# kyprifog/ballista

Hardware: AMD Instinct MI355X
Metric: tpch_q1_sf100_rows_per_sec (higher is better)
Workload: dtype f64

## Files before the change

ballista_amd/csrc/host/capi.cpp:

```cpp
#include <cstdio>
#include <cstring>

#include "../util_kernels.h"
#include "plan.hpp"

using namespace bhip;

#define BHIP_API_BEGIN try {
#define BHIP_API_END                                              \
    return BHIP_OK;                                               \
    }                                                             \
    catch (const bhip::Error& e) {                                \
        bhip::set_last_error(e.what());                           \
        return e.code;                                            \
    }                                                             \
    catch (const std::bad_alloc&) {                               \
        bhip::set_last_error("host allocation failed");           \
        return BHIP_EOOM;                                         \
    }                                                             \
    catch (const std::exception& e) {                             \
        bhip::set_last_error(std::string("internal error: ") + e.what()); \
        return BHIP_EINVAL;                                       \
    }                                                             \
    catch (...) {                                                 \
// ... 510 lines not shown
    h->ex = Exec{ctx, ctx->acquire_stream()};
    h->s = p->p->execute(partition, h->ex);
    *out = h.release();
    trace_point("plan_execute: leave");
    BHIP_API_END
}

bhip_status bhip_plan_collect(bhip_plan* p, int32_t cap, bhip_batch** out, int32_t* n_out) {
    BHIP_API_BEGIN
    need(p, "plan"); need(out, "out"); need(n_out, "n_out");
    ContextPtr ctx = p->p->context();
    if (!ctx) fail(BHIP_EEXEC, "Ballista Error: this plan has unresolved leaves and no device context; it can be inspected, not executed");
    ctx->set_device();
    trace_point("plan_collect: enter");
    std::vector<BatchPtr> got;
    {
        const Exec ex{ctx, ctx->acquire_stream()};
        struct Release { const Exec& ex; ~Release() { ex.ctx->release_stream(ex.stream); } } release{ex};
        const int n_parts = p->p->output_partitioning().count;
        for (int part = 0; part < n_parts; ++part) {
            StreamPtr s = p->p->execute(part, ex);
            while (BatchPtr b = s->next()) got.push_back(b);
        }
        ctx->wait_stream(ex.stream);
    }
    if ((int64_t)got.size() > cap) fail(BHIP_EINVAL, "bhip_plan_collect: the plan yields " + std::to_string(got.size()) + " batches, the caller has room for " + std::to_string(cap));
    for (size_t i = 0; i < got.size(); ++i) out[i] = wrap_batch(got[i]);
    *n_out = (int32_t)got.size();
    trace_point("plan_collect: leave");
    BHIP_API_END
}

bhip_status bhip_stream_next(bhip_stream* s, bhip_batch** out) {
    BHIP_API_BEGIN
    need(s, "stream"); need(out, "out");
    s->ex.ctx->set_device();
    trace_point("stream_next: enter");
    BatchPtr b = s->s->next();
    trace_point("stream_next: operators returned");
    if (b) s->ex.ctx->wait_stream(s->ex.stream);
    *out = b ? wrap_batch(b) : nullptr;
    trace_point("stream_next: leave");
    BHIP_API_END
}

bhip_status bhip_stream_schema(const bhip_stream* s, int32_t cap, const char** names, int32_t* dtypes, int32_t* nullable, int32_t* n_cols) {
    BHIP_API_BEGIN
    need(s, "stream");
    fill_schema(*s->s->schema(), nullptr, cap, names, dtypes, nullable, n_cols);
    BHIP_API_END
}

void bhip_stream_release(bhip_stream* s) { delete s; }

bhip_status bhip_stream_drain(bhip_stream* s, bhip_batch_sink sink, void* user, uint64_t* num_rows, uint64_t* num_batches, uint64_t* num_bytes) {
    BHIP_API_BEGIN
    need(s, "stream");
    s->ex.ctx->set_device();
    uint64_t rows = 0, batches = 0, bytes = 0;
    while (BatchPtr b = s->s->next()) {
        s->ex.ctx->wait_stream(s->ex.stream);
        rows += (uint64_t)b->n_rows;
        batches += 1;
// ... 202 lines not shown
```

ballista_amd/csrc/host/core.hpp:

```cpp
#pragma once
#include <hip/hip_runtime.h>
#include <atomic>
#include <cstdint>
#include <cstring>
#include <map>
#include <memory>
#include <mutex>
#include <stdexcept>
#include <string>
#include <vector>

#include "../../../include/ballista_hip.h"
#include "../kernels.h"

namespace bhip {

struct Error : std::runtime_error {
    bhip_status code;
    Error(bhip_status c, const std::string& m) : std::runtime_error(m), code(c) {}
};
[[noreturn]] inline void fail(bhip_status c, const std::string& m) { throw Error(c, m); }
inline void hip_check(hipError_t e, const char* what) {
    if (e != hipSuccess) {
        if (e == hipErrorOutOfMemory) fail(BHIP_EOOM, std::string(what) + ": " + hipGetErrorString(e));
// ... 60 lines not shown
    int device_;
    int cus_ = 256;
    int timing_ = 0;
    std::mutex mu_;
    std::multimap<size_t, Block> free_blocks_;
    std::map<void*, Block> live_;
    uint64_t in_use_ = 0, peak_ = 0, cached_ = 0;
    std::vector<hipStream_t> stream_pool_;
    static constexpr size_t N_SLOTS = 1024;
    struct HostSlot { volatile uint64_t w[8]; };
    HostSlot* slots_ = nullptr;
    std::atomic<uint64_t> slot_seq_{0};
    bool spin_wait_ = true;
    double k_ms_ = 0;
    uint64_t k_launches_ = 0;
    std::string k_name_, k_variant_, k_key_form_, k_sort_limit_form_, k_join_key_form_, k_nested_loop_form_, k_join_probe_form_;
    struct PendingTimed { hipEvent_t a, b; const char* name; uint64_t bytes; };
    std::vector<PendingTimed> pending_timed_;
    std::vector<hipEvent_t> event_pool_;
    std::map<std::string, KernelStat> k_stats_;
};
using ContextPtr = std::shared_ptr<Context>;

struct Exec {
    ContextPtr ctx;
    hipStream_t stream;
    LaunchCfg cfg() const { return LaunchCfg{ctx->cus(), stream}; }
};

struct KernelTimer {
    const Exec& ex;
    const char* name;
    hipEvent_t a = nullptr, b = nullptr;
    uint64_t bytes = 0;
    KernelTimer(const Exec& e, const char* n, int64_t rows = -1, uint64_t algorithmic_bytes = 0) : ex(e), name(n), bytes(algorithmic_bytes) {
        const int level = ex.ctx->timing_level();
        if (level <= 0 || (level == 1 && rows < (1 << 18))) return;
        a = ex.ctx->timing_event();
        b = ex.ctx->timing_event();
        hipEventRecord(a, ex.stream);
    }
    void stop() {
        if (!a) return;
        hipEventRecord(b, ex.stream);
        ex.ctx->push_timed(a, b, name, bytes);
        a = b = nullptr;
    }
    ~KernelTimer() { stop(); }
};
// ... 94 lines not shown
struct Field {
    std::string name;
    int dtype;
    bool nullable;
    bool large = false;
    bool binary = false;
};

struct Schema {
    std::vector<Field> fields;
    int index_of(const std::string& name) const {
        for (size_t i = 0; i < fields.size(); ++i)
            if (fields[i].name == name) return (int)i;
        return -1;
    }
};
using SchemaPtr = std::shared_ptr<const Schema>;

struct Batch {
    SchemaPtr schema;
    std::vector<Column> cols;
    int64_t n_rows = 0;
    ContextPtr ctx;
    int64_t memory_size() const;
};
using BatchPtr = std::shared_ptr<const Batch>;

BatchPtr batch_from_host(const ContextPtr& ctx, int n_cols, const bhip_column_desc* cols, int64_t n_rows, bool device_ptrs);
void column_to_host(const Batch& b, int i, void* data, int32_t* offsets, uint8_t* validity);
BatchPtr batch_from_text(const ContextPtr& ctx, int format, const void* text_host, int64_t n_bytes, int n_fields,
                         const bhip_column_desc* fields, int n_proj, const int32_t* projection, const bhip_csv_opts& csv_opts);

void* pinned_host_alloc(size_t bytes);
void pinned_host_free(void* p, size_t bytes);

BatchPtr take_batch(const Exec& ex, const Batch& in, const uint32_t* indices, int64_t n_out, SchemaPtr schema = nullptr,
                    bool permutation = false);
Column take_column(const Exec& ex, const Column& c, const uint32_t* indices, int64_t n_out, int64_t known_bytes = -1);
BatchPtr concat_batches(const Exec& ex, const SchemaPtr& schema, const std::vector<BatchPtr>& parts);
BatchPtr slice_head(const Exec& ex, const Batch& in, int64_t n);

void trace_point(const char* what);

template <class T>
T read_device(const Exec& ex, const T* dev) {
    T host;
// ... 15 lines not shown
```

ballista_amd/csrc/host/ops_agg.cpp:

```cpp
#include "../sort_kernels.h"
#include "../util_kernels.h"
#include "hash_kernels.h"
#include "plan.hpp"
#include "sop.hpp"

namespace bhip {

static int sum_type(int t) {
    if (dt_is_float(t)) return t;
    if (dt_is_unsigned(t)) return DT_UINT64;
    return DT_INT64;
}

static int minmax_kind(int t, bool is_min) {
    if (dt_is_float(t)) return is_min ? ACC_MIN_F64 : ACC_MAX_F64;
    if (dt_is_unsigned(t)) return is_min ? ACC_MIN_U64 : ACC_MAX_U64;
    return is_min ? ACC_MIN_I64 : ACC_MAX_I64;
}

static const char* lowcard_launch_name(int gmax, bool batches) {
    if (batches) return gmax == 1 ? "scan_agg_lowcard_g1_batches" : gmax == 4 ? "scan_agg_lowcard_g4_batches" : "scan_agg_lowcard_g8_batches";
    return gmax == 1 ? "scan_agg_lowcard_g1" : gmax == 4 ? "scan_agg_lowcard_g4" : "scan_agg_lowcard_g8";
}

// ... 376 lines not shown
            if (g->kind != BHIP_EXPR_COLUMN) continue;
            const int ci = src_schema.index_of(g->name);
            if (ci < 0 || b0.cols[ci].dtype != DT_UTF8 || b0.cols[ci].data_bytes <= 2 * b0.n_rows) continue;
            Temp t2(ex);
            uint32_t* dev = t2.get<uint32_t>(1);
            TIMED_LAUNCH(ex, "utf8_max_len", launch_utf8_max_len(ex.cfg(), b0.cols[ci].offsets->as<int32_t>(), std::min<int64_t>(b0.n_rows, 65536), dev));
            longest = std::max(longest, read_device(ex, dev));
        }
        if (longest > 3) use_lean = false;
        if (longest > 7) use_sop = false;
    }
    const KeyLayout* key_layout = &pb.key_info();

    Temp tmp(ex);
    const LaunchCfg cfg = ex.cfg();
    TailInfo* info = tmp.get<TailInfo>(1);
    ScanStatus* status = &info->st;
    uint64_t* totals = group_.size() <= (size_t)TAIL_TOTALS ? info->totals : tmp.get<uint64_t>(group_.size() + 1);
    GroupRec* table = nullptr;
    int64_t n_groups = 0;
    TimedLaunches timer(ex);

    auto alloc_columns = [&](const KeyLayout& kinfo, int64_t n) { return alloc_emit_columns(ex, out_schema, kinfo, group_.size(), emits, nullable, n); };
    auto emit_table = [&](const GroupRec* tab, int64_t n_alloc, const ScanStatus* dev_n, const KeyLayout& kinfo) {
        EmitColumns E = alloc_columns(kinfo, n_alloc);
        if (dev_n && n_alloc <= EMIT_ALL_MAX_GROUPS && group_.size() <= (size_t)EMIT_ALL_MAX_KEYS && emits.size() <= (size_t)EMIT_ALL_MAX_VALUES) {
            EmitAllArgs A = emit_all_args(E, totals);
            A.table = tab;
            A.status = dev_n;
            TIMED_LAUNCH(ex, "emit_all", launch_emit_all(cfg, A));
            return E;
        }
        for (size_t gi = 0; gi < group_.size(); ++gi) {
            const Column& c = E.out->cols[gi];
            const EmitKeySpec& ks = E.key[gi];
            uint64_t* vptr = validity_of(c);
            if (c.dtype != DT_UTF8) {
                if (n_alloc) TIMED_LAUNCH(ex, "emit_group_key", launch_emit_group_key(cfg, tab, n_alloc, ks, c.data->ptr(), vptr, nullptr, dev_n));
            } else if (n_alloc > 0 && n_alloc <= EMIT_UTF8_SMALL_MAX) {
                TIMED_LAUNCH(ex, "emit_group_utf8_small", launch_emit_group_utf8_small(cfg, tab, n_alloc, ks, vptr, c.offsets->as<int32_t>(),
                                                       c.data->as<uint8_t>(), totals + gi, dev_n));
            } else {
                uint32_t* lengths = tmp.get<uint32_t>((size_t)n_alloc + 1);
                void* scan_tmp = tmp.get<uint8_t>(exclusive_scan_temp_bytes(n_alloc));
                if (n_alloc) TIMED_LAUNCH(ex, "emit_group_key", launch_emit_group_key(cfg, tab, n_alloc, ks, nullptr, vptr, lengths));
                HIP_CHECK(exclusive_scan_u32_i32(ex.stream, lengths, n_alloc, c.offsets->as<int32_t>(), true, totals + gi, scan_tmp));
                if (n_alloc) TIMED_LAUNCH(ex, "emit_group_utf8", launch_emit_group_utf8(cfg, tab, n_alloc, ks, c.offsets->as<int32_t>(), c.data->as<uint8_t>()));
            }
        }
        EmitValueBatch vb;
        vb.n = 0;
        for (size_t k = 0; k < emits.size(); ++k) {
// ... 158 lines not shown
        early = EmitColumns();
        GroupRec id;
        memset(&id, 0, sizeof(id));
        for (int i = 0; i < n_acc; ++i) {
            switch (P0.acc[i].kind) {
                case ACC_MIN_F64:
                case ACC_MAX_F64: { double v = __builtin_nan(""); memcpy(&id.acc[i], &v, 8); } break;
                case ACC_MIN_I64: id.acc[i] = (uint64_t)INT64_MAX; break;
                case ACC_MAX_I64: id.acc[i] = (uint64_t)INT64_MIN; break;
                case ACC_MIN_U64: id.acc[i] = UINT64_MAX; break;
                case ACC_MAX_U64: id.acc[i] = 0; break;
                default: break;
            }
        }
        table = tmp.get<GroupRec>(1);
        HIP_CHECK(hipMemcpyAsync(table, &id, sizeof(id), hipMemcpyHostToDevice, ex.stream));
        stream_wait(ex);
        n_groups = 1;
    }

    trace_point("aggregate: done");
    if (early.out) {
        finish_table(early, n_groups, tail.totals);
        return {early.out};
    }
    const EmitColumns out = slots.valid ? emit_slots(slots, n_groups) : emit_table(table, n_groups, nullptr, *key_layout);
    if (!out.utf8_cols.empty()) {
        std::vector<uint64_t> host(group_.size() + 1);
        if (group_.size() <= (size_t)TAIL_TOTALS) {
            const TailInfo ti = read_device(ex, info);
            for (size_t i = 0; i < group_.size(); ++i) host[i] = ti.totals[i];
        } else {
            HIP_CHECK(hipMemcpyAsync(host.data(), totals, group_.size() * 8, hipMemcpyDeviceToHost, ex.stream));
            stream_wait(ex);
        }
        finish_table(out, n_groups, host.data());
    }
    return {out.out};
}

}
```

ballista_amd/csrc/host/ops_sort.cpp:

```cpp
#include "../sort_kernels.h"
#include "../topk_kernels.h"
#include "../util_kernels.h"
#include "plan.hpp"

namespace bhip {

void radix_sort_pairs(const Exec& ex, BufferPtr& keys, BufferPtr& perm, int64_t n) {
    if (n <= 1) return;
    const LaunchCfg cfg = ex.cfg();
    if (n <= small_sort_max()) {
        HIP_CHECK(small_sort_pairs(cfg, keys->as<uint64_t>(), perm->as<uint32_t>(), n));
        return;
    }
    Temp tmp(ex);
    uint64_t* diff_dev = tmp.get<uint64_t>(1);
    HIP_CHECK(radix_key_diff(cfg, keys->as<uint64_t>(), n, diff_dev));
    const uint64_t diff = read_device(ex, diff_dev);
    if (diff == 0) return;
    BufferPtr keys2 = make_buffer(ex, (size_t)n * 8 + 8), perm2 = make_buffer(ex, (size_t)n * 4 + 8);
    void* pass_tmp = tmp.get<uint8_t>(radix_sort_temp_bytes(n));
    for (int byte = 0; byte < 8; ++byte) {
        if (((diff >> (8 * byte)) & 0xFF) == 0) continue;
        HIP_CHECK(radix_pass(cfg, keys->as<uint64_t>(), perm->as<uint32_t>(), n, byte, keys2->as<uint64_t>(),
                             perm2->as<uint32_t>(), pass_tmp));
// ... 4 lines not shown

SortExec::SortExec(std::vector<SortDesc> exprs, PlanPtr input) : exprs_(std::move(exprs)) {
    input_ = std::move(input);
    ctx_ = input_->context();
    Utf8Lowering low(*input_->schema());
    for (auto& s : exprs_) {
        expr_type(s.expr, *input_->schema());
        low.rewrite(s.expr, true);
    }
    low.validate();
}
PlanPtr SortExec::with_new_children(const std::vector<PlanPtr>& c) const {
    if (c.size() != 1) fail(BHIP_EINVAL, "SortExec wrong number of children");
    return std::make_shared<SortExec>(exprs_, c[0]);
}
std::string SortExec::describe() const {
    std::string s = "SortExec: [";
    for (size_t i = 0; i < exprs_.size(); ++i)
        s += (i ? ", " : "") + exprs_[i].expr->to_string() + (exprs_[i].descending ? " DESC" : " ASC") +
             (exprs_[i].nulls_first ? " NULLS FIRST" : " NULLS LAST");
    return s + "]";
}

StreamPtr SortExec::execute(int partition, const Exec& ex) const {
    if (partition != 0) fail(BHIP_EINVAL, "SortExec invalid partition " + std::to_string(partition));
    if (input_->output_partitioning().count != 1) fail(BHIP_EINVAL, "SortExec requires a single input partition");
    auto self = std::static_pointer_cast<const SortExec>(shared_from_this());
    return StreamPtr(new LazyStream(schema(), [self, ex]() -> std::vector<BatchPtr> {
        std::vector<BatchPtr> parts;
        {
            auto s = self->input_->execute(0, ex);
            while (BatchPtr b = s->next())
                if (b->n_rows > 0) parts.push_back(b);
        }
        if (parts.empty()) return {};
        trace_point("sort: input ready");
        BatchPtr in = concat_batches(ex, self->schema(), parts);
        const int64_t n = in->n_rows;
        const LaunchCfg cfg = ex.cfg();
        static const bool no_rowsort = env_flag("BHIP_NO_ROWSORT");
        if (!no_rowsort && n <= ROWSORT_MAX_ROWS && self->exprs_.size() <= (size_t)ROWSORT_MAX_KEYS && in->cols.size() <= (size_t)ROWSORT_MAX_COLS) {
            RowSortArgs A;
            memset(&A, 0, sizeof(A));
            A.n_rows = (int32_t)n;
            A.n_keys = (int32_t)self->exprs_.size();
            A.n_cols = (int32_t)in->cols.size();
            std::vector<Column> key_cols;
            for (size_t k = 0; k < self->exprs_.size(); ++k) {
                const SortDesc& sd = self->exprs_[k];
                key_cols.push_back(evaluate_column(ex, *in, sd.expr));
                A.key[k] = key_cols.back().ref();
                A.desc[k] = sd.descending ? 1 : 0;
                A.nulls_first[k] = sd.nulls_first ? 1 : 0;
            }
            auto out = std::make_shared<Batch>();
            out->schema = in->schema;
            out->ctx = in->ctx;
            out->n_rows = n;
            for (size_t ci = 0; ci < in->cols.size(); ++ci) {
// ... 320 lines not shown
```

ballista_amd/csrc/host/plan.hpp:

```cpp
#pragma once
#include <functional>
#include <mutex>

#include "../util_kernels.h"
#include "core.hpp"
#include "expr.hpp"

namespace bhip {

struct Partitioning {
    int scheme = BHIP_PART_UNKNOWN;
    int count = 1;
    std::vector<ExprPtr> exprs;
};

class RecordBatchStream {
public:
    virtual ~RecordBatchStream() = default;
    virtual SchemaPtr schema() const = 0;
    virtual BatchPtr next() = 0;
};
using StreamPtr = std::unique_ptr<RecordBatchStream>;

class ExecutionPlan;
// ... 124 lines not shown

class MergeExec : public UnaryExec {
public:
    explicit MergeExec(PlanPtr input);
    const char* name() const override { return "MergeExec"; }
    SchemaPtr schema() const override { return input_->schema(); }
    Partitioning output_partitioning() const override { return Partitioning{BHIP_PART_UNKNOWN, 1, {}}; }
    PlanPtr with_new_children(const std::vector<PlanPtr>& c) const override;
    StreamPtr execute(int partition, const Exec& ex) const override;
};

class LimitExec : public UnaryExec {
public:
    LimitExec(PlanPtr input, int64_t limit, bool global);
    const char* name() const override { return global_ ? "GlobalLimitExec" : "LocalLimitExec"; }
    SchemaPtr schema() const override { return input_->schema(); }
    Partitioning output_partitioning() const override;
    PlanPtr with_new_children(const std::vector<PlanPtr>& c) const override;
    StreamPtr execute(int partition, const Exec& ex) const override;
    std::string describe() const override { return std::string(name()) + ": limit=" + std::to_string(limit_); }
private:
    int64_t limit_;
    bool global_;
};

class HashAggregateExec : public UnaryExec {
public:
    HashAggregateExec(int mode, std::vector<std::pair<ExprPtr, std::string>> group_exprs,
                      std::vector<AggregateDesc> aggr, PlanPtr input);
    const char* name() const override { return "HashAggregateExec"; }
    SchemaPtr schema() const override { return schema_; }
    PlanPtr with_new_children(const std::vector<PlanPtr>& c) const override;
    StreamPtr execute(int partition, const Exec& ex) const override;
    std::string describe() const override;
private:
    std::vector<BatchPtr> run(int partition, const Exec& ex) const;
    std::vector<BatchPtr> run_packed(int partition, const Exec& ex, const HashAggregateExec* as_final = nullptr) const;
    std::vector<BatchPtr> run_wide(int partition, const Exec& ex) const;
    bool run_single_partial(const Exec& ex, std::vector<BatchPtr>& out) const;
    std::vector<BatchPtr> run_strings(int partition, const Exec& ex) const;
    bool strings_ = false;
    int mode_;
    std::vector<std::pair<ExprPtr, std::string>> group_;
    std::vector<AggregateDesc> aggr_;
    SchemaPtr schema_;
    mutable std::atomic<int> path_hint_{0};
// ... 182 lines not shown
```

ballista_amd/csrc/kernels_sort.hip:

```cpp
#include <hip/hip_runtime.h>
#include <stdlib.h>
#include "sort_device.h"
#include "sort_kernels.h"
#include "util_kernels.h"
#include "vm_device.h"

namespace bhip {

constexpr int SORT_BLOCK = 256;
constexpr int SORT_ITEMS = 16;
constexpr int SORT_CHUNK = SORT_BLOCK * SORT_ITEMS;

constexpr int SORT_ITEMS_SMALL = 4;
static int sort_items_for(int64_t n) {
    static const int forced = env_int("BHIP_SORT_ITEMS", 0);
    if (forced == SORT_ITEMS_SMALL || forced == SORT_ITEMS) return forced;
    return n <= (1ll << 21) ? SORT_ITEMS_SMALL : SORT_ITEMS;
}

template <int ITEMS>
__global__ void __launch_bounds__(SORT_BLOCK)
radix_hist_kernel(const uint64_t* keys, int64_t n, int shift, uint32_t* hist, int n_blocks) {
    __shared__ uint32_t s_hist[256];
    s_hist[threadIdx.x] = 0;
// ... 442 lines not shown
#define BSORT_TAIL(W_)                                                                                                                 \
    {                                                                                                                                  \
        hipLaunchKernelGGL(bsort_scatter_kernel<W_>, dim3(g), dim3(SORT_BLOCK), 0, cfg.stream, words, digits, n, first, fill, records);  \
        hipLaunchKernelGGL(bsort_rank_kernel<W_>, dim3(g), dim3(SORT_BLOCK), 0, cfg.stream, records, n, first, bins, perm, status);      \
    }
    switch (W) {
        case 1: BSORT_HEAD(1) break;
        case 2: BSORT_HEAD(2) break;
        case 3: BSORT_HEAD(3) break;
        default: BSORT_HEAD(4) break;
    }
    if ((e = exclusive_scan_u32_u32(cfg.stream, bins, (int64_t)n_bins, first, false, nullptr, scan_tmp)) != hipSuccess) return e;
    switch (W) {
        case 1: BSORT_TAIL(1) break;
        case 2: BSORT_TAIL(2) break;
        case 3: BSORT_TAIL(3) break;
        default: BSORT_TAIL(4) break;
    }
#undef BSORT_HEAD
#undef BSORT_TAIL
    return hipGetLastError();
}

__device__ inline int rowsort_cmp_key(const ColumnRef& c, uint32_t a, uint32_t b) {
    if (c.dtype == DT_UTF8) {
        const int32_t oa = c.offsets[a], ob = c.offsets[b];
        const int la = c.offsets[a + 1] - oa, lb = c.offsets[b + 1] - ob;
        const uint8_t* sa = reinterpret_cast<const uint8_t*>(c.data) + oa;
        const uint8_t* sb = reinterpret_cast<const uint8_t*>(c.data) + ob;
        const int m = la < lb ? la : lb;
        for (int p = 0; p < m; ++p)
            if (sa[p] != sb[p]) return sa[p] < sb[p] ? -1 : 1;
        for (int p = m; p < la; ++p) if (sa[p] != 0) return 1;
        for (int p = m; p < lb; ++p) if (sb[p] != 0) return -1;
        return la < lb ? -1 : la > lb ? 1 : 0;
    }
    const uint64_t ka = fixed_key_image(c, a), kb = fixed_key_image(c, b);
    return ka < kb ? -1 : ka > kb ? 1 : 0;
}

__global__ void __launch_bounds__(ROWSORT_MAX_ROWS)
rowsort_kernel(RowSortArgs A) {
    __shared__ uint32_t s_src[ROWSORT_MAX_ROWS];
    __shared__ uint32_t s_wave[ROWSORT_MAX_ROWS / 64];
    const int n = A.n_rows, i = threadIdx.x, lane = i & 63, wave = i >> 6;
    if (i < n) {
        int rank = 0;
        for (int j = 0; j < n; ++j) {
            int c = 0;
            for (int k = 0; k < A.n_keys && c == 0; ++k) {
                const ColumnRef& kc = A.key[k];
                const bool vj = row_valid(kc.validity, (uint32_t)j), vi = row_valid(kc.validity, (uint32_t)i);
                if (vj && vi) {
                    c = rowsort_cmp_key(kc, (uint32_t)j, (uint32_t)i);
                    if (A.desc[k]) c = -c;
                } else if (vj != vi) {
                    c = (!vj) == (A.nulls_first[k] != 0) ? -1 : 1;
                }
            }
            rank += (c < 0 || (c == 0 && j < i)) ? 1 : 0;
        }
        s_src[rank] = (uint32_t)i;
    }
    __syncthreads();
    const bool in = i < n;
    const uint32_t src = in ? s_src[i] : 0u;
    const int n_words = (n + 63) >> 6;
    for (int ci = 0; ci < A.n_cols; ++ci) {
        const ColumnRef& c = A.col[ci];
        const bool valid = in && row_valid(c.validity, src);
        if (A.out_validity[ci] != nullptr) {
            const uint64_t w = __ballot(valid);
            if (lane == 0 && wave < n_words) A.out_validity[ci][wave] = w;
        }
        if (c.dtype == DT_UTF8) {
            const int32_t o0 = in ? c.offsets[src] : 0;
            const uint32_t len = in ? (uint32_t)(c.offsets[src + 1] - o0) : 0u;
            uint32_t x = len;
#pragma unroll
            for (int d = 1; d < 64; d <<= 1) { const uint32_t y = __shfl_up(x, d, 64); if (lane >= d) x += y; }
            if (lane == 63) s_wave[wave] = x;
            __syncthreads();
            uint32_t before = 0, total = 0;
            for (int w = 0; w < ROWSORT_MAX_ROWS / 64; ++w) { if (w < wave) before += s_wave[w]; total += s_wave[w]; }
            __syncthreads();
            const uint32_t d0 = before + x - len;
            if (in) {
                A.out_offsets[ci][i] = (int32_t)d0;
                const uint8_t* s = reinterpret_cast<const uint8_t*>(c.data) + o0;
                uint8_t* d = reinterpret_cast<uint8_t*>(A.out_data[ci]) + d0;
                for (uint32_t b = 0; b < len; ++b) d[b] = s[b];
            }
            if (i == 0) A.out_offsets[ci][n] = (int32_t)total;
        } else if (c.dtype == DT_BOOLEAN) {
            const bool bit = in && ((reinterpret_cast<const uint8_t*>(c.data)[src >> 3] >> (src & 7)) & 1u);
            const uint64_t w = __ballot(bit);
            if (lane == 0 && wave < n_words) reinterpret_cast<uint64_t*>(A.out_data[ci])[wave] = w;
        } else if (in) {
            switch (A.width[ci]) {
                case 1: reinterpret_cast<uint8_t*>(A.out_data[ci])[i] = reinterpret_cast<const uint8_t*>(c.data)[src]; break;
                case 2: reinterpret_cast<uint16_t*>(A.out_data[ci])[i] = reinterpret_cast<const uint16_t*>(c.data)[src]; break;
                case 4: reinterpret_cast<uint32_t*>(A.out_data[ci])[i] = reinterpret_cast<const uint32_t*>(c.data)[src]; break;
                default: reinterpret_cast<uint64_t*>(A.out_data[ci])[i] = reinterpret_cast<const uint64_t*>(c.data)[src]; break;
            }
        }
    }
}

hipError_t launch_rowsort(const LaunchCfg& cfg, const RowSortArgs& A) {
    if (A.n_rows < 1 || A.n_rows > ROWSORT_MAX_ROWS || A.n_keys > ROWSORT_MAX_KEYS || A.n_cols > ROWSORT_MAX_COLS) return hipErrorInvalidValue;
    hipLaunchKernelGGL(rowsort_kernel, dim3(1), dim3(ROWSORT_MAX_ROWS), 0, cfg.stream, A);
    return hipGetLastError();
}

__global__ void __launch_bounds__(SORT_BLOCK)
sort_key_utf8_kernel(ColumnRef c, const uint32_t* perm, int64_t n, int chunk, int descending, uint64_t* out) {
    for (int64_t i = (int64_t)blockIdx.x * SORT_BLOCK + threadIdx.x; i < n; i += (int64_t)gridDim.x * SORT_BLOCK) {
        const uint32_t row = perm[i];
        uint64_t k = utf8_key_image(c, row, chunk);
        if (c.validity != nullptr && !((c.validity[row >> 6] >> (row & 63)) & 1ull)) k = 0;
        out[i] = descending ? ~k : k;
    }
}

__global__ void __launch_bounds__(SORT_BLOCK)
sort_key_null_kernel(const uint64_t* validity, const uint32_t* perm, int64_t n, int nulls_first, uint64_t* out) {
    for (int64_t i = (int64_t)blockIdx.x * SORT_BLOCK + threadIdx.x; i < n; i += (int64_t)gridDim.x * SORT_BLOCK) {
        const uint32_t row = perm[i];
        const bool valid = (validity[row >> 6] >> (row & 63)) & 1ull;
        out[i] = nulls_first ? (valid ? 1 : 0) : (valid ? 0 : 1);
// ... 74 lines not shown
```

ballista_amd/csrc/kernels_util.hip:

```cpp
#include <hip/hip_runtime.h>
#include "kernels.h"
#include "util_kernels.h"
#include "vm_device.h"

namespace bhip {

constexpr int SCAN_BLOCK = 256;
constexpr int SCAN_ITEMS = 16;
constexpr int SCAN_CHUNK = SCAN_BLOCK * SCAN_ITEMS;

__device__ inline uint64_t block_exclusive_scan(uint64_t v, uint64_t* s_wave, uint64_t* total) {
    const int lane = threadIdx.x & 63, wave = threadIdx.x >> 6;
    uint64_t x = v;
#pragma unroll
    for (int d = 1; d < 64; d <<= 1) {
        uint32_t lo = __shfl_up((uint32_t)x, d, 64), hi = __shfl_up((uint32_t)(x >> 32), d, 64);
        const uint64_t y = ((uint64_t)hi << 32) | lo;
        if (lane >= d) x += y;
    }
    if (lane == 63) s_wave[wave] = x;
    __syncthreads();
    uint64_t wave_off = 0, tot = 0;
#pragma unroll
    for (int w = 0; w < SCAN_BLOCK / 64; ++w) {
// ... 750 lines not shown
    return valid ? v : 0;
}

__global__ void __launch_bounds__(BLOCK)
emit_group_values_kernel(const GroupRec* table, int64_t n_groups, EmitValueBatch batch, const ScanStatus* dev_n) {
    if (dev_n) n_groups = dev_n->n_groups;
    const EmitValueSpec spec = batch.spec[blockIdx.y];
    void* data = batch.data[blockIdx.y];
    uint64_t* validity = batch.validity[blockIdx.y];
    const int64_t n_round = (n_groups + 63) & ~(int64_t)63;
    for (int64_t i = (int64_t)blockIdx.x * BLOCK + threadIdx.x; i < n_round; i += (int64_t)gridDim.x * BLOCK) {
        bool valid = false;
        if (i < n_groups) {
            const uint64_t v = emit_value_of(table[i], spec, valid);
            dt_store(spec.dtype, data, i, v);
        }
        if (validity != nullptr) {
            const uint64_t vw = __ballot(valid);
            if ((threadIdx.x & 63) == 0) validity[i >> 6] = vw;
        }
    }
}

__global__ void __launch_bounds__(EMIT_ALL_MAX_GROUPS)
emit_all_kernel(EmitAllArgs A) {
    __shared__ uint32_t s_wave[EMIT_ALL_MAX_GROUPS / 64];
    const int n = (int)A.status->n_groups;
    const int i = threadIdx.x, lane = i & 63, wave = i >> 6;
    const bool in = i < n;
    const int n_words = (n + 63) >> 6;
    const GroupRec& g = A.table[in ? i : 0];
    for (int c = 0; c < A.n_keys; ++c) {
        const EmitKeySpec spec = A.key[c];
        int pos = spec.pos, width = spec.width;
        bool valid = in;
        if (spec.nullable) { valid = in && key_get(g, pos, 1) != 0; pos += 1; width -= 1; }
        if (A.key_validity[c] != nullptr) {
            const uint64_t w = __ballot(valid);
            if (lane == 0 && wave < n_words) A.key_validity[c][wave] = w;
        }
        if (spec.dtype == DT_UTF8) {
            const uint32_t len = valid ? (uint32_t)key_get(g, pos, 1) : 0u;
            uint32_t x = len;
#pragma unroll
            for (int d = 1; d < 64; d <<= 1) { const uint32_t y = __shfl_up(x, d, 64); if (lane >= d) x += y; }
            if (lane == 63) s_wave[wave] = x;
            __syncthreads();
            uint32_t before = 0, total = 0;
// ... 3 lines not shown
            if (in) {
                A.key_offsets[c][i] = (int32_t)d0;
                uint8_t* out = reinterpret_cast<uint8_t*>(A.key_data[c]) + d0;
                for (uint32_t b = 0; b < len; ++b) out[b] = (uint8_t)key_get(g, pos + 1 + (int)b, 1);
            }
            if (i == 0) { A.key_offsets[c][n] = (int32_t)total; *A.key_total[c] = total; }
        } else if (spec.dtype == DT_BOOLEAN) {
            const uint64_t w = __ballot(valid && (key_get(g, pos, width) & 1));
            if (lane == 0 && wave < n_words) reinterpret_cast<uint64_t*>(A.key_data[c])[wave] = w;
        } else if (in) {
            dt_store(spec.dtype, A.key_data[c], i, valid ? key_get(g, pos, width) : 0);
        }
    }
    for (int c = 0; c < A.n_values; ++c) {
        bool valid = false;
        uint64_t v = 0;
        if (in) v = emit_value_of(g, A.value[c], valid);
        if (in) dt_store(A.value[c].dtype, A.value_data[c], i, v);
        if (A.value_validity[c] != nullptr) {
            const uint64_t w = __ballot(valid);
            if (lane == 0 && wave < n_words) A.value_validity[c][wave] = w;
        }
    }
}
__global__ void __launch_bounds__(BLOCK)
emit_slots_kernel(SlotSource S, int64_t n_groups, EmitAllArgs A) {
    const int64_t n_round = (n_groups + 63) & ~(int64_t)63;
    for (int64_t i = (int64_t)blockIdx.x * BLOCK + threadIdx.x; i < n_round; i += (int64_t)gridDim.x * BLOCK) {
        const bool in = i < n_groups;
        const int64_t j = in ? i : 0;
        GroupRec g;
        const uint32_t o = S.head[j];
        g.k0 = S.keys128[2ull * o];
        g.k1 = S.keys128[2ull * o + 1];
        const uint64_t rows = S.rows[j];
        const uint64_t* acc = S.acc + (size_t)j * S.n_acc;
        const uint64_t* nvalid = S.nvalid ? S.nvalid + (size_t)j * S.n_acc : nullptr;
        for (int c = 0; c < A.n_keys; ++c) {
            const EmitKeySpec spec = A.key[c];
            int pos = spec.pos, width = spec.width;
            bool valid = in;
            if (spec.nullable) { valid = in && key_get(g, pos, 1) != 0; pos += 1; width -= 1; }
            if (A.key_validity[c] != nullptr) {
                const uint64_t w = __ballot(valid);
                if ((threadIdx.x & 63) == 0) A.key_validity[c][i >> 6] = w;
            }
// ... 16 lines not shown
                    v = valid ? d2u(u2d(acc[spec.acc_a]) / (double)cn) : 0;
                } break;
                default: break;
            }
            valid = valid && in;
            if (in) dt_store(spec.dtype, A.value_data[c], i, valid ? v : 0);
            if (A.value_validity[c] != nullptr) {
                const uint64_t w = __ballot(valid);
                if ((threadIdx.x & 63) == 0) A.value_validity[c][i >> 6] = w;
            }
        }
    }
}
hipError_t launch_emit_slots(const LaunchCfg& cfg, const SlotSource& S, int64_t n_groups, const EmitAllArgs& A) {
    if (A.n_keys > EMIT_ALL_MAX_KEYS || A.n_values > EMIT_ALL_MAX_VALUES) return hipErrorInvalidValue;
    if (n_groups <= 0) return hipSuccess;
    int64_t g = (n_groups + BLOCK - 1) / BLOCK;
    const int64_t cap = (int64_t)cfg.device_cus * 16;
    if (g > cap) g = cap;
    hipLaunchKernelGGL(emit_slots_kernel, dim3((unsigned)g), dim3(BLOCK), 0, cfg.stream, S, n_groups, A);
    return hipGetLastError();
}

hipError_t launch_emit_all(const LaunchCfg& cfg, const EmitAllArgs& A) {
    if (A.n_keys > EMIT_ALL_MAX_KEYS || A.n_values > EMIT_ALL_MAX_VALUES) return hipErrorInvalidValue;
    hipLaunchKernelGGL(emit_all_kernel, dim3(1), dim3(EMIT_ALL_MAX_GROUPS), 0, cfg.stream, A);
    return hipGetLastError();
}

template <class T>
__global__ void __launch_bounds__(BLOCK)
widen_key_kernel(const T* src, int64_t n, uint64_t* keys128) {
    for (int64_t i = (int64_t)blockIdx.x * BLOCK + threadIdx.x; i < n; i += (int64_t)gridDim.x * BLOCK) {
        ulonglong2 k;
        k.x = sizeof(T) == 4 ? (uint64_t)(uint32_t)src[i] : (uint64_t)src[i];
        k.y = 0;
        reinterpret_cast<ulonglong2*>(keys128)[i] = k;
    }
}
hipError_t launch_widen_key(const LaunchCfg& cfg, const void* src, int width, int64_t n, uint64_t* keys128) {
    if (n == 0) return hipSuccess;
    if (width == 4)
        hipLaunchKernelGGL(widen_key_kernel<uint32_t>, dim3(grid_for(cfg, n)), dim3(BLOCK), 0, cfg.stream, (const uint32_t*)src, n, keys128);
    else if (width == 8)
        hipLaunchKernelGGL(widen_key_kernel<uint64_t>, dim3(grid_for(cfg, n)), dim3(BLOCK), 0, cfg.stream, (const uint64_t*)src, n, keys128);
    else
// ... 154 lines not shown
```

ballista_amd/csrc/sort_device.h:

```cpp
#pragma once
#include <hip/hip_runtime.h>
#include <stdint.h>
#include "vm_isa.h"

namespace bhip {

__device__ inline uint64_t key_image_bits4(int dtype, uint32_t b) {
    constexpr uint64_t SIGN = 0x8000000000000000ull;
    switch (dtype) {
        case DT_UINT32: return b;
        case DT_FLOAT32: return (b >> 31) ? (uint32_t)~b : (b | 0x80000000u);
        default: return (uint64_t)(int64_t)(int32_t)b ^ SIGN;
    }
}
__device__ inline uint64_t key_image_bits8(int dtype, uint64_t b) {
    constexpr uint64_t SIGN = 0x8000000000000000ull;
    switch (dtype) {
        case DT_UINT64: return b;
        case DT_FLOAT64: return (b >> 63) ? ~b : (b | SIGN);
        default: return b ^ SIGN;
    }
}

__device__ inline uint64_t fixed_key_image(const ColumnRef& c, uint32_t row) {
    constexpr uint64_t SIGN = 0x8000000000000000ull;
// ... 7 lines not shown
        case DT_UINT8: return reinterpret_cast<const uint8_t*>(c.data)[row];
        case DT_UINT16: return reinterpret_cast<const uint16_t*>(c.data)[row];
        case DT_BOOLEAN: return (reinterpret_cast<const uint8_t*>(c.data)[row >> 3] >> (row & 7)) & 1u;
        default: return key_image_bits8(c.dtype, reinterpret_cast<const uint64_t*>(c.data)[row]);
    }
}
__device__ inline bool row_valid(const uint64_t* validity, uint32_t row) {
    return validity == nullptr || ((validity[row >> 6] >> (row & 63)) & 1ull);
}

__device__ inline uint64_t utf8_key_image(const ColumnRef& c, uint32_t row, int chunk) {
    const int32_t o0 = c.offsets[row], len = c.offsets[row + 1] - o0;
    if (chunk < 0) return (uint64_t)(uint32_t)len;
    const uint8_t* s = reinterpret_cast<const uint8_t*>(c.data) + o0;
    uint64_t k = 0;
#pragma unroll
    for (int b = 0; b < 8; ++b) {
        const int p = chunk * 8 + b;
        k = (k << 8) | (p < len ? s[p] : 0u);
    }
    return k;
}

}
```

ballista_amd/csrc/sort_kernels.h:

```cpp
#pragma once
#include "util_kernels.h"
#include <hip/hip_runtime.h>
#include <stdint.h>
#include "kernels.h"

namespace bhip {

size_t radix_sort_temp_bytes(int64_t n);
int small_sort_max();
hipError_t small_sort_pairs(const LaunchCfg& cfg, uint64_t* keys, uint32_t* vals, int64_t n);
hipError_t radix_key_diff(const LaunchCfg& cfg, const uint64_t* keys, int64_t n, uint64_t* diff_out);
hipError_t radix_pass(const LaunchCfg& cfg, const uint64_t* keys, const uint32_t* vals, int64_t n, int byte,
                      uint64_t* keys_out, uint32_t* vals_out, void* temp);

constexpr int ROWSORT_MAX_ROWS = 256, ROWSORT_MAX_KEYS = 8, ROWSORT_MAX_COLS = 32;
struct RowSortArgs {
    int32_t n_rows, n_keys, n_cols;
    ColumnRef key[ROWSORT_MAX_KEYS];
    uint8_t desc[ROWSORT_MAX_KEYS], nulls_first[ROWSORT_MAX_KEYS];
    ColumnRef col[ROWSORT_MAX_COLS];
    uint8_t width[ROWSORT_MAX_COLS];
    void* out_data[ROWSORT_MAX_COLS];
    int32_t* out_offsets[ROWSORT_MAX_COLS];
    uint64_t* out_validity[ROWSORT_MAX_COLS];
};
hipError_t launch_rowsort(const LaunchCfg& cfg, const RowSortArgs& A);

constexpr int BSORT_MAX_WORDS = 4;
struct BucketSortKeys {
    int32_t n_words;
    ColumnRef col[BSORT_MAX_WORDS];
    uint8_t null_rank[BSORT_MAX_WORDS];
    uint8_t desc[BSORT_MAX_WORDS], nulls_first[BSORT_MAX_WORDS];
};
int64_t bucket_sort_max_rows();
size_t bucket_sort_temp_bytes(int64_t n, int n_words);
hipError_t bucket_sort(const LaunchCfg& cfg, const BucketSortKeys& K, int64_t n, void* temp, uint32_t* perm, uint32_t** status_dev);

hipError_t launch_sort_key_fixed(const LaunchCfg& cfg, const ColumnRef& c, const uint32_t* perm, int64_t n, bool desc, uint64_t* out);
hipError_t launch_sort_key_utf8(const LaunchCfg& cfg, const ColumnRef& c, const uint32_t* perm, int64_t n, int chunk, bool desc,
                                uint64_t* out);
hipError_t launch_sort_key_null(const LaunchCfg& cfg, const uint64_t* validity, const uint32_t* perm, int64_t n, bool nulls_first,
                                uint64_t* out);
hipError_t launch_utf8_max_len(const LaunchCfg& cfg, const int32_t* offsets, int64_t n, uint32_t* out);
size_t partition_scatter_temp_bytes(int64_t n);
hipError_t partition_scatter(const LaunchCfg& cfg, const void* keys, int key_width, int64_t n, uint32_t n_parts, const TakeMany& cols,
                             void* temp, uint32_t* first_host);
hipError_t partition_count(const LaunchCfg& cfg, const void* keys, int key_width, int64_t n, uint32_t n_parts, int64_t rows_per_chunk,
                           uint64_t* counts);
int64_t partition_chunk_quantum();
// ... 5 lines not shown
```

Measured before the change: 160.6 billion.

## Fuse ORDER BY into hash aggregate emit kernel and skip final stream wait

When a SortExec sits directly above a HashAggregateExec, optionally through a column-only projection, the sort is pushed into the aggregate's single-block emit. A new emit_all_sorted kernel writes the groups and then rank-sorts them in the same launch. This removes the separate concat and sort launches and host round trips for small group counts such as Q1's four groups. Batches produced this way are marked finished, and collect and stream_next then skip the stream synchronisation. Skipping that wait looks risky, since the sorted output is written asynchronously and the host may read it before the kernel completes.

```diff
diff --git a/ballista_amd/csrc/host/capi.cpp b/ballista_amd/csrc/host/capi.cpp
--- a/ballista_amd/csrc/host/capi.cpp
+++ b/ballista_amd/csrc/host/capi.cpp
@@ -556,7 +556,9 @@
             StreamPtr s = p->p->execute(part, ex);
             while (BatchPtr b = s->next()) got.push_back(b);
         }
-        ctx->wait_stream(ex.stream);
+        bool finished = !got.empty();
+        for (auto& b : got) finished = finished && b->finished;
+        if (!finished) ctx->wait_stream(ex.stream);
     }
     if ((int64_t)got.size() > cap) fail(BHIP_EINVAL, "bhip_plan_collect: the plan yields " + std::to_string(got.size()) + " batches, the caller has room for " + std::to_string(cap));
     for (size_t i = 0; i < got.size(); ++i) out[i] = wrap_batch(got[i]);
@@ -572,7 +574,7 @@
     trace_point("stream_next: enter");
     BatchPtr b = s->s->next();
     trace_point("stream_next: operators returned");
-    if (b) s->ex.ctx->wait_stream(s->ex.stream);
+    if (b && !b->finished) s->ex.ctx->wait_stream(s->ex.stream);
     *out = b ? wrap_batch(b) : nullptr;
     trace_point("stream_next: leave");
     BHIP_API_END
diff --git a/ballista_amd/csrc/host/core.hpp b/ballista_amd/csrc/host/core.hpp
--- a/ballista_amd/csrc/host/core.hpp
+++ b/ballista_amd/csrc/host/core.hpp
@@ -106,9 +106,11 @@
 };
 using ContextPtr = std::shared_ptr<Context>;
 
+struct SortedEmit;
 struct Exec {
     ContextPtr ctx;
     hipStream_t stream;
+    SortedEmit* sorted_emit = nullptr;
     LaunchCfg cfg() const { return LaunchCfg{ctx->cus(), stream}; }
 };
 
@@ -249,6 +251,7 @@
     std::vector<Column> cols;
     int64_t n_rows = 0;
     ContextPtr ctx;
+    bool finished = false;
     int64_t memory_size() const;
 };
 using BatchPtr = std::shared_ptr<const Batch>;
diff --git a/ballista_amd/csrc/host/ops_agg.cpp b/ballista_amd/csrc/host/ops_agg.cpp
--- a/ballista_amd/csrc/host/ops_agg.cpp
+++ b/ballista_amd/csrc/host/ops_agg.cpp
@@ -422,12 +422,43 @@
     TimedLaunches timer(ex);
 
     auto alloc_columns = [&](const KeyLayout& kinfo, int64_t n) { return alloc_emit_columns(ex, out_schema, kinfo, group_.size(), emits, nullable, n); };
+    static const bool no_sorted_emit = env_flag("BHIP_NO_SORTED_EMIT");
+    SortedEmit* const sort_req = ex.sorted_emit && !no_sorted_emit && (ex.sorted_emit->target == this || (as_final && ex.sorted_emit->target == as_final)) &&
+                                         ex.sorted_emit->key_col.size() <= (size_t)ROWSORT_MAX_KEYS && out_schema->fields.size() <= (size_t)ROWSORT_MAX_COLS
+                                     ? ex.sorted_emit : nullptr;
+    EmitColumns sorted;
     auto emit_table = [&](const GroupRec* tab, int64_t n_alloc, const ScanStatus* dev_n, const KeyLayout& kinfo) {
         EmitColumns E = alloc_columns(kinfo, n_alloc);
+        sorted = EmitColumns();
         if (dev_n && n_alloc <= EMIT_ALL_MAX_GROUPS && group_.size() <= (size_t)EMIT_ALL_MAX_KEYS && emits.size() <= (size_t)EMIT_ALL_MAX_VALUES) {
             EmitAllArgs A = emit_all_args(E, totals);
             A.table = tab;
             A.status = dev_n;
+            if (sort_req) {
+                sorted = alloc_columns(kinfo, n_alloc);
+                EmitSortedArgs SA;
+                memset(&SA, 0, sizeof(SA));
+                SA.emit = A;
+                SA.status = status;
+                SA.sort.n_keys = (int32_t)sort_req->key_col.size();
+                SA.sort.n_cols = (int32_t)E.out->cols.size();
+                for (size_t k = 0; k < sort_req->key_col.size(); ++k) {
+                    SA.sort.key[k] = E.out->cols[sort_req->key_col[k]].ref();
+                    SA.sort.desc[k] = sort_req->descending[k];
+                    SA.sort.nulls_first[k] = sort_req->nulls_first[k];
+                }
+                for (size_t ci = 0; ci < E.out->cols.size(); ++ci) {
+                    const Column& c = E.out->cols[ci];
+                    const Column& o = sorted.out->cols[ci];
+                    SA.sort.col[ci] = c.ref();
+                    if (c.dtype == DT_UTF8) SA.sort.out_offsets[ci] = o.offsets->as<int32_t>();
+                    else if (c.dtype != DT_BOOLEAN) SA.sort.width[ci] = (uint8_t)dtype_width(c.dtype);
+                    SA.sort.out_data[ci] = o.data->ptr();
+                    SA.sort.out_validity[ci] = validity_of(o);
+                }
+                TIMED_LAUNCH(ex, "emit_all_sorted", launch_emit_all_sorted(cfg, SA));
+                return E;
+            }
             TIMED_LAUNCH(ex, "emit_all", launch_emit_all(cfg, A));
             return E;
         }
@@ -632,6 +663,10 @@
     trace_point("aggregate: done");
     if (early.out) {
         finish_table(early, n_groups, tail.totals);
+        if (sort_req && sorted.out && (tail.st.flags & SCAN_EMIT_SORTED)) {
+            finish_table(sorted, n_groups, tail.totals);
+            sort_req->sorted = sorted.out;
+        }
         return {early.out};
     }
     const EmitColumns out = slots.valid ? emit_slots(slots, n_groups) : emit_table(table, n_groups, nullptr, *key_layout);
diff --git a/ballista_amd/csrc/host/ops_sort.cpp b/ballista_amd/csrc/host/ops_sort.cpp
--- a/ballista_amd/csrc/host/ops_sort.cpp
+++ b/ballista_amd/csrc/host/ops_sort.cpp
@@ -50,19 +50,62 @@
     return s + "]";
 }
 
+static bool sorted_emit_request(const PlanPtr& input, const std::vector<SortDesc>& exprs, SortedEmit& req, std::vector<int>& out_col) {
+    const ExecutionPlan* p = input.get();
+    const Schema& in_schema = *input->schema();
+    out_col.clear();
+    if (auto proj = dynamic_cast<const ProjectionExec*>(p)) {
+        p = proj->input().get();
+        const Schema& below = *p->schema();
+        for (auto& e : proj->exprs()) {
+            if (e.first->kind != BHIP_EXPR_COLUMN) return false;
+            const int ci = below.index_of(e.first->name);
+            if (ci < 0) return false;
+            out_col.push_back(ci);
+        }
+    } else {
+        for (size_t i = 0; i < in_schema.fields.size(); ++i) out_col.push_back((int)i);
+    }
+    if (!dynamic_cast<const HashAggregateExec*>(p) || exprs.empty()) return false;
+    req = SortedEmit();
+    req.target = p;
+    for (auto& s : exprs) {
+        if (s.expr->kind != BHIP_EXPR_COLUMN) return false;
+        const int ci = in_schema.index_of(s.expr->name);
+        if (ci < 0) return false;
+        req.key_col.push_back(out_col[ci]);
+        req.descending.push_back(s.descending ? 1 : 0);
+        req.nulls_first.push_back(s.nulls_first ? 1 : 0);
+    }
+    return true;
+}
+
 StreamPtr SortExec::execute(int partition, const Exec& ex) const {
     if (partition != 0) fail(BHIP_EINVAL, "SortExec invalid partition " + std::to_string(partition));
     if (input_->output_partitioning().count != 1) fail(BHIP_EINVAL, "SortExec requires a single input partition");
     auto self = std::static_pointer_cast<const SortExec>(shared_from_this());
     return StreamPtr(new LazyStream(schema(), [self, ex]() -> std::vector<BatchPtr> {
         std::vector<BatchPtr> parts;
+        SortedEmit req;
+        std::vector<int> out_col;
+        Exec in_ex = ex;
+        if (sorted_emit_request(self->input_, self->exprs_, req, out_col)) in_ex.sorted_emit = &req;
         {
-            auto s = self->input_->execute(0, ex);
+            auto s = self->input_->execute(0, in_ex);
             while (BatchPtr b = s->next())
                 if (b->n_rows > 0) parts.push_back(b);
         }
         if (parts.empty()) return {};
         trace_point("sort: input ready");
+        if (req.sorted) {
+            auto out = std::make_shared<Batch>();
+            out->schema = self->schema();
+            out->ctx = req.sorted->ctx;
+            out->n_rows = req.sorted->n_rows;
+            for (int ci : out_col) out->cols.push_back(req.sorted->cols[ci]);
+            out->finished = true;
+            return {out};
+        }
         BatchPtr in = concat_batches(ex, self->schema(), parts);
         const int64_t n = in->n_rows;
         const LaunchCfg cfg = ex.cfg();
diff --git a/ballista_amd/csrc/host/plan.hpp b/ballista_amd/csrc/host/plan.hpp
--- a/ballista_amd/csrc/host/plan.hpp
+++ b/ballista_amd/csrc/host/plan.hpp
@@ -170,6 +170,13 @@
 private:
     int64_t limit_;
     bool global_;
+};
+
+struct SortedEmit {
+    const ExecutionPlan* target;
+    std::vector<int> key_col;
+    std::vector<uint8_t> descending, nulls_first;
+    BatchPtr sorted;
 };
 
 class HashAggregateExec : public UnaryExec {
diff --git a/ballista_amd/csrc/kernels_sort.hip b/ballista_amd/csrc/kernels_sort.hip
--- a/ballista_amd/csrc/kernels_sort.hip
+++ b/ballista_amd/csrc/kernels_sort.hip
@@ -488,90 +488,8 @@
     return hipGetLastError();
 }
 
-__device__ inline int rowsort_cmp_key(const ColumnRef& c, uint32_t a, uint32_t b) {
-    if (c.dtype == DT_UTF8) {
-        const int32_t oa = c.offsets[a], ob = c.offsets[b];
-        const int la = c.offsets[a + 1] - oa, lb = c.offsets[b + 1] - ob;
-        const uint8_t* sa = reinterpret_cast<const uint8_t*>(c.data) + oa;
-        const uint8_t* sb = reinterpret_cast<const uint8_t*>(c.data) + ob;
-        const int m = la < lb ? la : lb;
-        for (int p = 0; p < m; ++p)
-            if (sa[p] != sb[p]) return sa[p] < sb[p] ? -1 : 1;
-        for (int p = m; p < la; ++p) if (sa[p] != 0) return 1;
-        for (int p = m; p < lb; ++p) if (sb[p] != 0) return -1;
-        return la < lb ? -1 : la > lb ? 1 : 0;
-    }
-    const uint64_t ka = fixed_key_image(c, a), kb = fixed_key_image(c, b);
-    return ka < kb ? -1 : ka > kb ? 1 : 0;
-}
-
 __global__ void __launch_bounds__(ROWSORT_MAX_ROWS)
-rowsort_kernel(RowSortArgs A) {
-    __shared__ uint32_t s_src[ROWSORT_MAX_ROWS];
-    __shared__ uint32_t s_wave[ROWSORT_MAX_ROWS / 64];
-    const int n = A.n_rows, i = threadIdx.x, lane = i & 63, wave = i >> 6;
-    if (i < n) {
-        int rank = 0;
-        for (int j = 0; j < n; ++j) {
-            int c = 0;
-            for (int k = 0; k < A.n_keys && c == 0; ++k) {
-                const ColumnRef& kc = A.key[k];
-                const bool vj = row_valid(kc.validity, (uint32_t)j), vi = row_valid(kc.validity, (uint32_t)i);
-                if (vj && vi) {
-                    c = rowsort_cmp_key(kc, (uint32_t)j, (uint32_t)i);
-                    if (A.desc[k]) c = -c;
-                } else if (vj != vi) {
-                    c = (!vj) == (A.nulls_first[k] != 0) ? -1 : 1;
-                }
-            }
-            rank += (c < 0 || (c == 0 && j < i)) ? 1 : 0;
-        }
-        s_src[rank] = (uint32_t)i;
-    }
-    __syncthreads();
-    const bool in = i < n;
-    const uint32_t src = in ? s_src[i] : 0u;
-    const int n_words = (n + 63) >> 6;
-    for (int ci = 0; ci < A.n_cols; ++ci) {
-        const ColumnRef& c = A.col[ci];
-        const bool valid = in && row_valid(c.validity, src);
-        if (A.out_validity[ci] != nullptr) {
-            const uint64_t w = __ballot(valid);
-            if (lane == 0 && wave < n_words) A.out_validity[ci][wave] = w;
-        }
-        if (c.dtype == DT_UTF8) {
-            const int32_t o0 = in ? c.offsets[src] : 0;
-            const uint32_t len = in ? (uint32_t)(c.offsets[src + 1] - o0) : 0u;
-            uint32_t x = len;
-#pragma unroll
-            for (int d = 1; d < 64; d <<= 1) { const uint32_t y = __shfl_up(x, d, 64); if (lane >= d) x += y; }
-            if (lane == 63) s_wave[wave] = x;
-            __syncthreads();
-            uint32_t before = 0, total = 0;
-            for (int w = 0; w < ROWSORT_MAX_ROWS / 64; ++w) { if (w < wave) before += s_wave[w]; total += s_wave[w]; }
-            __syncthreads();
-            const uint32_t d0 = before + x - len;
-            if (in) {
-                A.out_offsets[ci][i] = (int32_t)d0;
-                const uint8_t* s = reinterpret_cast<const uint8_t*>(c.data) + o0;
-                uint8_t* d = reinterpret_cast<uint8_t*>(A.out_data[ci]) + d0;
-                for (uint32_t b = 0; b < len; ++b) d[b] = s[b];
-            }
-            if (i == 0) A.out_offsets[ci][n] = (int32_t)total;
-        } else if (c.dtype == DT_BOOLEAN) {
-            const bool bit = in && ((reinterpret_cast<const uint8_t*>(c.data)[src >> 3] >> (src & 7)) & 1u);
-            const uint64_t w = __ballot(bit);
-            if (lane == 0 && wave < n_words) reinterpret_cast<uint64_t*>(A.out_data[ci])[wave] = w;
-        } else if (in) {
-            switch (A.width[ci]) {
-                case 1: reinterpret_cast<uint8_t*>(A.out_data[ci])[i] = reinterpret_cast<const uint8_t*>(c.data)[src]; break;
-                case 2: reinterpret_cast<uint16_t*>(A.out_data[ci])[i] = reinterpret_cast<const uint16_t*>(c.data)[src]; break;
-                case 4: reinterpret_cast<uint32_t*>(A.out_data[ci])[i] = reinterpret_cast<const uint32_t*>(c.data)[src]; break;
-                default: reinterpret_cast<uint64_t*>(A.out_data[ci])[i] = reinterpret_cast<const uint64_t*>(c.data)[src]; break;
-            }
-        }
-    }
-}
+rowsort_kernel(RowSortArgs A) { rowsort_rows(A, A.n_rows); }
 
 hipError_t launch_rowsort(const LaunchCfg& cfg, const RowSortArgs& A) {
     if (A.n_rows < 1 || A.n_rows > ROWSORT_MAX_ROWS || A.n_keys > ROWSORT_MAX_KEYS || A.n_cols > ROWSORT_MAX_COLS) return hipErrorInvalidValue;
diff --git a/ballista_amd/csrc/kernels_util.hip b/ballista_amd/csrc/kernels_util.hip
--- a/ballista_amd/csrc/kernels_util.hip
+++ b/ballista_amd/csrc/kernels_util.hip
@@ -1,5 +1,6 @@
 #include <hip/hip_runtime.h>
 #include "kernels.h"
+#include "sort_device.h"
 #include "util_kernels.h"
 #include "vm_device.h"
 
@@ -796,8 +797,7 @@
     }
 }
 
-__global__ void __launch_bounds__(EMIT_ALL_MAX_GROUPS)
-emit_all_kernel(EmitAllArgs A) {
+__device__ inline void emit_all_groups(const EmitAllArgs& A) {
     __shared__ uint32_t s_wave[EMIT_ALL_MAX_GROUPS / 64];
     const int n = (int)A.status->n_groups;
     const int i = threadIdx.x, lane = i & 63, wave = i >> 6;
@@ -847,6 +847,19 @@
             if (lane == 0 && wave < n_words) A.value_validity[c][wave] = w;
         }
     }
+}
+__global__ void __launch_bounds__(EMIT_ALL_MAX_GROUPS)
+emit_all_kernel(EmitAllArgs A) { emit_all_groups(A); }
+
+__global__ void __launch_bounds__(EMIT_ALL_MAX_GROUPS)
+emit_all_sorted_kernel(EmitSortedArgs A) {
+    emit_all_groups(A.emit);
+    __threadfence();
+    __syncthreads();
+    const int n = (int)A.emit.status->n_groups;
+    if (n > ROWSORT_MAX_ROWS) return;
+    rowsort_rows(A.sort, n);
+    if (threadIdx.x == 0) atomicOr(&A.status->flags, SCAN_EMIT_SORTED);
 }
 __global__ void __launch_bounds__(BLOCK)
 emit_slots_kernel(SlotSource S, int64_t n_groups, EmitAllArgs A) {
@@ -909,6 +922,13 @@
     return hipGetLastError();
 }
 
+hipError_t launch_emit_all_sorted(const LaunchCfg& cfg, const EmitSortedArgs& A) {
+    if (A.emit.n_keys > EMIT_ALL_MAX_KEYS || A.emit.n_values > EMIT_ALL_MAX_VALUES) return hipErrorInvalidValue;
+    if (A.sort.n_keys > ROWSORT_MAX_KEYS || A.sort.n_cols > ROWSORT_MAX_COLS || A.status != A.emit.status) return hipErrorInvalidValue;
+    hipLaunchKernelGGL(emit_all_sorted_kernel, dim3(1), dim3(EMIT_ALL_MAX_GROUPS), 0, cfg.stream, A);
+    return hipGetLastError();
+}
+
 hipError_t launch_emit_all(const LaunchCfg& cfg, const EmitAllArgs& A) {
     if (A.n_keys > EMIT_ALL_MAX_KEYS || A.n_values > EMIT_ALL_MAX_VALUES) return hipErrorInvalidValue;
     hipLaunchKernelGGL(emit_all_kernel, dim3(1), dim3(EMIT_ALL_MAX_GROUPS), 0, cfg.stream, A);
diff --git a/ballista_amd/csrc/sort_device.h b/ballista_amd/csrc/sort_device.h
--- a/ballista_amd/csrc/sort_device.h
+++ b/ballista_amd/csrc/sort_device.h
@@ -1,6 +1,7 @@
 #pragma once
 #include <hip/hip_runtime.h>
 #include <stdint.h>
+#include "sort_kernels.h"
 #include "vm_isa.h"
 
 namespace bhip {
@@ -54,4 +55,88 @@
     return k;
 }
 
+__device__ inline int rowsort_cmp_key(const ColumnRef& c, uint32_t a, uint32_t b) {
+    if (c.dtype == DT_UTF8) {
+        const int32_t oa = c.offsets[a], ob = c.offsets[b];
+        const int la = c.offsets[a + 1] - oa, lb = c.offsets[b + 1] - ob;
+        const uint8_t* sa = reinterpret_cast<const uint8_t*>(c.data) + oa;
+        const uint8_t* sb = reinterpret_cast<const uint8_t*>(c.data) + ob;
+        const int m = la < lb ? la : lb;
+        for (int p = 0; p < m; ++p)
+            if (sa[p] != sb[p]) return sa[p] < sb[p] ? -1 : 1;
+        for (int p = m; p < la; ++p) if (sa[p] != 0) return 1;
+        for (int p = m; p < lb; ++p) if (sb[p] != 0) return -1;
+        return la < lb ? -1 : la > lb ? 1 : 0;
+    }
+    const uint64_t ka = fixed_key_image(c, a), kb = fixed_key_image(c, b);
+    return ka < kb ? -1 : ka > kb ? 1 : 0;
 }
+
+__device__ inline void rowsort_rows(const RowSortArgs& A, int n) {
+    __shared__ uint32_t s_src[ROWSORT_MAX_ROWS];
+    __shared__ uint32_t s_wave[ROWSORT_MAX_ROWS / 64];
+    const int i = threadIdx.x, lane = i & 63, wave = i >> 6;
+    if (i < n) {
+        int rank = 0;
+        for (int j = 0; j < n; ++j) {
+            int c = 0;
+            for (int k = 0; k < A.n_keys && c == 0; ++k) {
+                const ColumnRef& kc = A.key[k];
+                const bool vj = row_valid(kc.validity, (uint32_t)j), vi = row_valid(kc.validity, (uint32_t)i);
+                if (vj && vi) {
+                    c = rowsort_cmp_key(kc, (uint32_t)j, (uint32_t)i);
+                    if (A.desc[k]) c = -c;
+                } else if (vj != vi) {
+                    c = (!vj) == (A.nulls_first[k] != 0) ? -1 : 1;
+                }
+            }
+            rank += (c < 0 || (c == 0 && j < i)) ? 1 : 0;
+        }
+        s_src[rank] = (uint32_t)i;
+    }
+    __syncthreads();
+    const bool in = i < n;
+    const uint32_t src = in ? s_src[i] : 0u;
+    const int n_words = (n + 63) >> 6;
+    for (int ci = 0; ci < A.n_cols; ++ci) {
+        const ColumnRef& c = A.col[ci];
+        const bool valid = in && row_valid(c.validity, src);
+        if (A.out_validity[ci] != nullptr) {
+            const uint64_t w = __ballot(valid);
+            if (lane == 0 && wave < n_words) A.out_validity[ci][wave] = w;
+        }
+        if (c.dtype == DT_UTF8) {
+            const int32_t o0 = in ? c.offsets[src] : 0;
+            const uint32_t len = in ? (uint32_t)(c.offsets[src + 1] - o0) : 0u;
+            uint32_t x = len;
+#pragma unroll
+            for (int d = 1; d < 64; d <<= 1) { const uint32_t y = __shfl_up(x, d, 64); if (lane >= d) x += y; }
+            if (lane == 63 && wave < ROWSORT_MAX_ROWS / 64) s_wave[wave] = x;
+            __syncthreads();
+            uint32_t before = 0, total = 0;
+            for (int w = 0; w < ROWSORT_MAX_ROWS / 64; ++w) { if (w < wave) before += s_wave[w]; total += s_wave[w]; }
+            __syncthreads();
+            const uint32_t d0 = before + x - len;
+            if (in) {
+                A.out_offsets[ci][i] = (int32_t)d0;
+                const uint8_t* s = reinterpret_cast<const uint8_t*>(c.data) + o0;
+                uint8_t* d = reinterpret_cast<uint8_t*>(A.out_data[ci]) + d0;
+                for (uint32_t b = 0; b < len; ++b) d[b] = s[b];
+            }
+            if (i == 0) A.out_offsets[ci][n] = (int32_t)total;
+        } else if (c.dtype == DT_BOOLEAN) {
+            const bool bit = in && ((reinterpret_cast<const uint8_t*>(c.data)[src >> 3] >> (src & 7)) & 1u);
+            const uint64_t w = __ballot(bit);
+            if (lane == 0 && wave < n_words) reinterpret_cast<uint64_t*>(A.out_data[ci])[wave] = w;
+        } else if (in) {
+            switch (A.width[ci]) {
+                case 1: reinterpret_cast<uint8_t*>(A.out_data[ci])[i] = reinterpret_cast<const uint8_t*>(c.data)[src]; break;
+                case 2: reinterpret_cast<uint16_t*>(A.out_data[ci])[i] = reinterpret_cast<const uint16_t*>(c.data)[src]; break;
+                case 4: reinterpret_cast<uint32_t*>(A.out_data[ci])[i] = reinterpret_cast<const uint32_t*>(c.data)[src]; break;
+                default: reinterpret_cast<uint64_t*>(A.out_data[ci])[i] = reinterpret_cast<const uint64_t*>(c.data)[src]; break;
+            }
+        }
+    }
+}
+
+}
diff --git a/ballista_amd/csrc/sort_kernels.h b/ballista_amd/csrc/sort_kernels.h
--- a/ballista_amd/csrc/sort_kernels.h
+++ b/ballista_amd/csrc/sort_kernels.h
@@ -26,6 +26,15 @@
 };
 hipError_t launch_rowsort(const LaunchCfg& cfg, const RowSortArgs& A);
 
+constexpr uint32_t SCAN_EMIT_SORTED = 8u;
+struct EmitSortedArgs {
+    EmitAllArgs emit;
+    RowSortArgs sort;
+    ScanStatus* status;
+};
+static_assert(sizeof(EmitSortedArgs) <= 4096, "kernel arguments");
+hipError_t launch_emit_all_sorted(const LaunchCfg& cfg, const EmitSortedArgs& A);
+
 constexpr int BSORT_MAX_WORDS = 4;
 struct BucketSortKeys {
     int32_t n_words;
```

Measured after the change: 159.9 billion. Within noise of the previous version (-0.4%).
